# MattJBorowski1991/QuantizedMHA

Measured on AMD Instinct MI355X. Metric: attention-fwd TFLOPS + ms/call, B16 H16 N4096 d64 (fp16 & int8), higher is better.
Workload: dtype int8; 1 GPU; fa_tc_int8_b attention forward (BASELINE config 4); variant=fa_tc_int8_b, B_per_gpu=16, H=16, N=4096, d=64, d_model=1024, global_batch=16, parallelism=batch-shard x1 (no collective in the timed step; all-gather reported separately)

## Files before the change

### include/launchers.h

```cpp
#ifndef QMHA_LAUNCHERS_H
#define QMHA_LAUNCHERS_H

#include <stddef.h>
#include <stdint.h>

#ifdef __cplusplus
extern "C" {
#endif

typedef enum {
    QMHA_FA = 0,
    QMHA_FA_TC_V1A = 1,
    QMHA_FA_TC_INT8_B = 2,
    QMHA_UNFUSED = 3,
    QMHA_FA_MFMA = 4,
    QMHA_FA_TC_INT8_PT = 5
} qmha_variant_t;

enum {
    QMHA_OK = 0,
    QMHA_ERR_INVALID = 1,
    QMHA_ERR_HIP = 2,
    QMHA_ERR_NOMEM = 3,
    QMHA_ERR_NOSYS = 4
// ... 23 lines not shown
                       int variant);

int qmha_quantize_int8(const float *X, int B, int N, int d_model, int h, int8_t *Xi, float *scales, int layout,
                       void *stream);

int qmha_debug_qk_int32(const float *Q, const float *K, int N, int d_model, int h, int head, int32_t *S);

int qmha_debug_fa_int8_dump(const float *Q, const float *K, const float *V, float *O, int B, int N, int d_model,
                            int h, int32_t *S, int8_t *Qi, float *sQ);

int qmha_debug_fa_int8_pt_dump(const float *Q, const float *K, const float *V, float *O, int B, int N, int d_model,
                               int h, int32_t *S, int8_t *Qi, float *sQ);

int64_t qmha_debug_set_pt_wait(int64_t ticks);

int qmha_variant_from_name(const char *name);
const char *qmha_variant_name(int variant);
const char *qmha_status_string(int status);
const char *qmha_version(void);
const char *qmha_last_error(void);

void qmha_profile_enable(int on);
int qmha_set_overlap_chunks(int n);
int qmha_profile_collect(double *main_ms, long long *launches, double *prepass_ms);

void qmha_release_workspaces(void);

#ifdef __cplusplus
}
#endif
#endif
```

### quantizedmha_amd/_lib.py

```python
from __future__ import annotations

import ctypes
import os
import threading

HERE = os.path.dirname(os.path.abspath(__file__))
LIB_DIR = os.path.join(HERE, "lib")
LIB_PATH = os.environ.get("QMHA_LIB_PATH") or os.path.join(LIB_DIR, "libqmha.so")

VARIANTS = {"fa": 0, "fa_tc_v1a": 1, "fa_tc_int8_b": 2, "unfused": 3, "fa_mfma": 4, "fa_tc_int8_pt": 5}
DEFAULT_KERNEL = "fa_tc_int8_b"
QMHA_OK = 0
QMHA_FLAG_CAUSAL = 1

_i, _sz, _vp, _cp = ctypes.c_int, ctypes.c_size_t, ctypes.c_void_p, ctypes.c_char_p
SIGNATURES = {
    "solve": (None, [_vp, _vp, _vp, _vp, _i, _i, _i]),
    "qmha_solve_ex": (_i, [_vp, _vp, _vp, _vp, _i, _i, _i, _i, _i, _vp]),
    "qmha_solve_opts": (_i, [_vp, _vp, _vp, _vp, _i, _i, _i, _i, _i, ctypes.c_uint, _vp, _sz, _vp]),
    "qmha_solve_rect": (_i, [_vp, _vp, _vp, _vp, _i, _i, _i, _i, _i, _i, ctypes.c_uint, _vp, _sz, _vp]),
    "qmha_workspace_size": (_sz, [_i, _i, _i, _i, _i]),
    "qmha_solve_ws": (_i, [_vp, _vp, _vp, _vp, _i, _i, _i, _i, _i, _vp, _sz, _vp]),
    "qmha_solve_variant": (_i, [_vp, _vp, _vp, _vp, _i, _i, _i, _i]),
    "qmha_quantize_int8": (_i, [_vp, _i, _i, _i, _i, _vp, _vp, _i, _vp]),
    "qmha_debug_qk_int32": (_i, [_vp, _vp, _i, _i, _i, _i, _vp]),
    "qmha_debug_fa_int8_dump": (_i, [_vp, _vp, _vp, _vp, _i, _i, _i, _i, _vp, _vp, _vp]),
    "qmha_debug_fa_int8_pt_dump": (_i, [_vp, _vp, _vp, _vp, _i, _i, _i, _i, _vp, _vp, _vp]),
    "qmha_variant_from_name": (_i, [_cp]),
    "qmha_variant_name": (_cp, [_i]),
    "qmha_status_string": (_cp, [_i]),
    "qmha_version": (_cp, []),
    "qmha_last_error": (_cp, []),
    "qmha_profile_enable": (None, [_i]),
    "qmha_set_overlap_chunks": (_i, [_i]),
    "qmha_debug_set_pt_wait": (ctypes.c_longlong, [ctypes.c_longlong]),
    "qmha_profile_collect": (_i, [ctypes.POINTER(ctypes.c_double), ctypes.POINTER(ctypes.c_longlong),
                                  ctypes.POINTER(ctypes.c_double)]),
    "qmha_release_workspaces": (None, []),
}

_lock = threading.Lock()
_lib = None


class QMHAError(RuntimeError):
    pass


def load(path: str = LIB_PATH):
    global _lib
    with _lock:
        if _lib is None:
            if not os.path.exists(path):
                raise QMHAError(f"native library {path} not found: run `python tools/build.py` "
                                "(quantizedmha_amd has no non-HIP fallback)")
            lib = ctypes.CDLL(path)
            for name, (res, args) in SIGNATURES.items():
# ... 18 lines not shown
```

### quantizedmha_amd/csrc/qmha_api.cpp

```cpp
#include <hip/hip_runtime.h>

#include <atomic>
#include <cstdio>
#include <cstdlib>
#include <cstring>
#include <map>
#include <memory>
#include <mutex>
#include <string>
#include <thread>
#include <utility>
#include <vector>

#include "../../include/launchers.h"
#include "qmha_kernels.hpp"

#define QMHA_VERSION_STRING "qmha-mi355x 0.1.0 (gfx950)"

namespace {

thread_local std::string g_last_error;

int fail(int status, std::string why) {
    g_last_error = std::move(why);
// ... 122 lines not shown
int timed(Marks* marks, hipStream_t s, const char* what, Launch&& launch) {
    int st = marks ? mark(*marks, s, true) : QMHA_OK;
    if (st != QMHA_OK) return st;
    QMHA_HIP_TRY(launch(), what);
    return marks ? mark(*marks, s, false) : QMHA_OK;
}

struct WsKey {
    int dev;
    void* stream;
    std::thread::id tid;
    bool operator<(const WsKey& o) const {
        if (dev != o.dev) return dev < o.dev;
        if (stream != o.stream) return stream < o.stream;
        return tid < o.tid;
    }
};
struct WsSlot {
    std::mutex lease;
    void* ptr = nullptr;
    size_t bytes = 0;
    std::vector<std::pair<void*, hipEvent_t>> retired;
    hipStream_t side = nullptr;
    hipEvent_t start = nullptr;
    std::vector<hipEvent_t> ready;
};
std::mutex g_ws_mu;
std::map<WsKey, std::unique_ptr<WsSlot>> g_ws;

void reap_retired(WsSlot& s, bool wait) {
    auto it = s.retired.begin();
    while (it != s.retired.end()) {
        if (wait) (void)hipEventSynchronize(it->second);
        else if (hipEventQuery(it->second) != hipSuccess) {
            ++it;
            continue;
        }
        (void)hipEventDestroy(it->second);
        (void)hipFree(it->first);
        it = s.retired.erase(it);
    }
}

struct WsLease {
    std::unique_lock<std::mutex> lk;
    WsSlot* slot = nullptr;
    void* ptr = nullptr;
// ... 21 lines not shown
            const hipError_t e = hipEventRecord(ev, stream);
            if (e != hipSuccess) {
                (void)hipEventDestroy(ev);
                return hip_fail(e, "hipEventRecord");
            }
            s.retired.emplace_back(s.ptr, ev);
            s.ptr = nullptr;
            s.bytes = 0;
        }
        const size_t alloc = qmha::align_up(need + need / 8, 1 << 20);
        if (hipMalloc(&s.ptr, alloc) != hipSuccess) {
            s.ptr = nullptr;
            return fail(QMHA_ERR_NOMEM, "hipMalloc of workspace failed");
        }
        s.bytes = alloc;
    }
    out->ptr = s.ptr;
    return QMHA_OK;
}

constexpr int kMaxChunks = 16;
std::atomic<int> g_overlap_chunks{-1};

int clamp_chunks(int c) { return c < 1 ? 1 : (c > kMaxChunks ? kMaxChunks : c); }

int overlap_chunks(int B) {
    int c = g_overlap_chunks.load();
    if (c < 0) {
#ifdef QMHA_ABLATION
        const char* e = std::getenv("QMHA_OVERLAP_CHUNKS");
        c = clamp_chunks(e ? std::atoi(e) : 1);
#else
        c = 1;
#endif
        g_overlap_chunks.store(c);
    }
    return c > B ? B : c;
}

int ensure_side(WsSlot& s, int nchunks) {
    if (!s.side) QMHA_HIP_TRY(hipStreamCreateWithFlags(&s.side, hipStreamNonBlocking), "hipStreamCreate");
    if (!s.start) QMHA_HIP_TRY(hipEventCreateWithFlags(&s.start, hipEventDisableTiming), "hipEventCreate");
    while ((int)s.ready.size() < nchunks) {
        hipEvent_t e = nullptr;
        QMHA_HIP_TRY(hipEventCreateWithFlags(&e, hipEventDisableTiming), "hipEventCreate");
        s.ready.push_back(e);
    }
    return QMHA_OK;
}

struct Chunk {
    size_t b0;
    int nb;
};

template <class Pre, class Main>
int run_chunked(int B, hipStream_t stream, WsSlot& slot, Marks* pre_m, Marks* main_m, const char* pre_what, Pre&& pre,
                const char* main_what, Main&& main) {
    const int nc = overlap_chunks(B);
    hipStream_t pre_s = stream;
    if (nc > 1) {
        int st = ensure_side(slot, nc);
        if (st != QMHA_OK) return st;
        QMHA_HIP_TRY(hipEventRecord(slot.start, stream), "hipEventRecord");
        QMHA_HIP_TRY(hipStreamWaitEvent(slot.side, slot.start, 0), "hipStreamWaitEvent");
        pre_s = slot.side;
    }
    Chunk ch[kMaxChunks];
    for (int c = 0; c < nc; ++c) {
        const long long b0 = (long long)B * c / nc, b1 = (long long)B * (c + 1) / nc;
        ch[c] = Chunk{(size_t)b0, (int)(b1 - b0)};
        int st = timed(pre_m, pre_s, pre_what, [&] { return pre(ch[c], pre_s); });
        if (st != QMHA_OK) return st;
        if (nc > 1) QMHA_HIP_TRY(hipEventRecord(slot.ready[c], pre_s), "hipEventRecord");
    }
    for (int c = 0; c < nc; ++c) {
        if (nc > 1) QMHA_HIP_TRY(hipStreamWaitEvent(stream, slot.ready[c], 0), "hipStreamWaitEvent");
        int st = timed(main_m, stream, main_what, [&] { return main(ch[c]); });
        if (st != QMHA_OK) return st;
    }
    return QMHA_OK;
}

qmha::Int8Workspace int8_slice(qmha::Int8Workspace w, size_t b0, int N, int H, int D) {
    const size_t e = b0 * H * N * D, g = b0 * H * (N / 32);
    w.Ki += e, w.Vh += e, w.sK += g, w.sV += g;
    return w;
}
qmha::F16Workspace f16_slice(qmha::F16Workspace w, size_t b0, int N, int H, int D) {
    const size_t e = b0 * H * N * D;
    w.Kh += e, w.Vt += e;
    return w;
}

int run(const float* Q, const float* K, const float* V, float* O, int B, int Nq, int N, int d_model, int h, int variant,
        unsigned flags, void* ws, WsSlot& slot, hipStream_t stream) {
    const int D = d_model / h;
    const bool causal = flags & QMHA_FLAG_CAUSAL;
    const bool rect = Nq != N;
    const bool masked = causal || rect;
    bool prof;
    {
        std::lock_guard<std::mutex> lk(g_prof_mu);
        prof = g_prof_on;
    }
    ProfRec rec;
    Marks *pre_m = prof ? &rec.pre : nullptr, *main_m = prof ? &rec.main : nullptr;
    const size_t slab = (size_t)N * d_model, qslab = (size_t)Nq * d_model;
    int st;
    switch (variant) {
        case QMHA_FA_TC_INT8_B: {
            const qmha::Int8Workspace w8 = qmha::int8_carve(ws, B, N, h, D);
            st = run_chunked(
                B, stream, slot, pre_m, main_m, "quant_int8 launch",
                [&](Chunk c, hipStream_t s) {
                    const qmha::Int8Workspace w = int8_slice(w8, c.b0, N, h, D);
                    return qmha::launch_quant_int8(Q + c.b0 * qslab, K + c.b0 * slab, V + c.b0 * slab, w, w.Vh, 1,
                                                   c.nb, N, h, D, d_model, s, 1);
                },
                rect ? "fa_int8 rect launch" : causal ? "fa_int8 causal launch" : "fa_int8 launch",
                [&](Chunk c) {
                    const qmha::Int8Workspace w = int8_slice(w8, c.b0, N, h, D);
                    const float* q = Q + c.b0 * qslab;
                    float* o = O + c.b0 * qslab;
                    return masked ? qmha::launch_fa_int8_masked_main(w, q, o, c.nb, Nq, N, h, D, d_model, causal, stream)
                                  : qmha::launch_fa_int8_main(w, q, o, c.nb, N, h, D, d_model, stream);
                });
            break;
        }
        case QMHA_FA_TC_V1A: {
            const qmha::F16Workspace w16 = qmha::f16_carve(ws, B, N, h, D);
            st = run_chunked(
                B, stream, slot, pre_m, main_m, "convert_f16 launch",
                [&](Chunk c, hipStream_t s) {
                    return qmha::launch_convert_f16(Q + c.b0 * qslab, K + c.b0 * slab, V + c.b0 * slab,
                                                    f16_slice(w16, c.b0, N, h, D), c.nb, N, h, D, d_model, s);
                },
                rect ? "fa_f16 rect launch" : causal ? "fa_f16 causal launch" : "fa_f16 launch",
                [&](Chunk c) {
                    const qmha::F16Workspace w = f16_slice(w16, c.b0, N, h, D);
                    const float* q = Q + c.b0 * qslab;
                    float* o = O + c.b0 * qslab;
                    return masked ? qmha::launch_fa_f16_masked_main(w, q, o, c.nb, Nq, N, h, D, d_model, causal, stream)
                                  : qmha::launch_fa_f16_main(w, q, o, c.nb, N, h, D, d_model, stream);
                });
            break;
        }
        case QMHA_FA_TC_INT8_PT: {
            const qmha::Int8Workspace w = qmha::int8_pt_carve(ws, B, N, h, D);
            st = timed(pre_m, stream, "quant_int8_pt launch",
                       [&] { return qmha::launch_quant_int8_pt(Q, K, V, w, B, N, h, D, d_model, stream); });
            if (st == QMHA_OK)
                st = timed(main_m, stream, "fa_int8_pt launch",
                           [&] { return qmha::launch_fa_int8_pt_main(w, Q, O, B, N, h, D, d_model, stream); });
            break;
        }
        case QMHA_FA:
        case QMHA_FA_MFMA:
            st = timed(main_m, stream, "fa_f32 launch",
                       [&] { return qmha::launch_fa_f32(Q, K, V, O, B, N, h, D, d_model, variant == QMHA_FA_MFMA, stream); });
            break;
        case QMHA_UNFUSED:
            st = timed(main_m, stream, "unfused launch",
                       [&] { return qmha::launch_unfused(Q, K, V, O, ws, B, N, h, D, d_model, stream); });
            break;
        default: return fail(QMHA_ERR_INVALID, "unknown variant");
    }
// ... 130 lines not shown
            return fail(QMHA_ERR_NOSYS, "layout 2 (per-tensor scales) is built for d = " + d_list(have) + " only");
        WsLease ws;
        st = lease_workspace(qmha::pt_slice_sync_bytes(B, h), (hipStream_t)stream, &ws);
        if (st != QMHA_OK) return st;
        qmha::Int8Workspace w{};
        w.Ki = Xi;
        w.sK = scales;
        w.slice_sync = static_cast<uint32_t*>(ws.ptr);
        QMHA_HIP_TRY(qmha::launch_quant_int8_pt_rows(X, w, B, N, h, D, d_model, (hipStream_t)stream), "quant_int8_pt launch");
        return QMHA_OK;
    }
    qmha::Int8Workspace w{};
    void* vout = nullptr;
    int v_mode = 1, role = 0;
    if (layout == 0) {
        w.Qi = Xi;
        w.sQ = scales;
    } else {
        vout = Xi;
        v_mode = 0;
        w.sV = scales;
        role = 2;
    }
    QMHA_HIP_TRY(qmha::launch_quant_int8(X, X, X, w, vout, v_mode, B, N, h, D, d_model, (hipStream_t)stream, role, 1),
                 "quant_int8 launch");
    return QMHA_OK;
}

int qmha_debug_qk_int32(const float* Q, const float* K, int N, int d_model, int h, int head, int32_t* S) {
    int D = 0;
    int st = check_shape(Q, K, Q, S, 1, N, d_model, h, QMHA_FA_TC_INT8_B, &D);
    if (st != QMHA_OK) return st;
    if (head < 0 || head >= h) return fail(QMHA_ERR_INVALID, "head out of range");
    return debug_run(qmha::int8_workspace_bytes(1, N, h, D, true), [&](void* ws) -> int {
        const qmha::Int8Workspace w = qmha::int8_carve(ws, 1, N, h, D, true);
        QMHA_HIP_TRY(qmha::launch_quant_int8(Q, K, Q, w, w.Vh, 1, 1, N, h, D, d_model, nullptr), "quant_int8 launch");
        QMHA_HIP_TRY(qmha::launch_debug_qk_int32(w, N, D, head, S, nullptr), "debug_qk launch");
        return QMHA_OK;
    });
}

int qmha_debug_fa_int8_dump(const float* Q, const float* K, const float* V, float* O, int B, int N, int d_model,
                            int h, int32_t* S, int8_t* Qi, float* sQ) {
    int D = 0;
    int st = check_shape(Q, K, V, O, B, N, d_model, h, QMHA_FA_TC_INT8_B, &D);
    if (st != QMHA_OK) return st;
    if (!S || !Qi || !sQ || ((D == 32 || D == 64 || D == 128) && N < 64))
// ... 34 lines not shown
const char* qmha_variant_name(int v) {
    const VariantRow* r = find_variant(v);
    return r ? r->name : "unknown";
}

const char* qmha_status_string(int s) {
    switch (s) {
        case QMHA_OK: return "ok";
        case QMHA_ERR_INVALID: return "invalid argument";
        case QMHA_ERR_HIP: return "HIP error";
        case QMHA_ERR_NOMEM: return "out of device memory";
        case QMHA_ERR_NOSYS: return "not supported";
        default: return "unknown status";
    }
}

const char* qmha_version(void) { return QMHA_VERSION_STRING; }

const char* qmha_last_error(void) { return g_last_error.c_str(); }

int64_t qmha_debug_set_pt_wait(int64_t ticks) { return qmha::set_pt_wait_ticks(ticks); }

int qmha_set_overlap_chunks(int n) {
    const int prev = overlap_chunks(1 << 30);
    g_overlap_chunks.store(clamp_chunks(n));
    return prev;
}

void qmha_profile_enable(int on) {
    std::lock_guard<std::mutex> lk(g_prof_mu);
    g_prof_on = on != 0;
}

int qmha_profile_collect(double* main_ms, long long* launches, double* prepass_ms) {
    std::vector<ProfRec> recs;
    {
        std::lock_guard<std::mutex> lk(g_prof_mu);
        recs.swap(g_prof_recs);
    }
    double tm = 0.0, tp = 0.0;
    for (auto& r : recs) {
        for (auto* v : {&r.main, &r.pre}) {
            for (auto& pr : *v) {
                QMHA_HIP_TRY(hipEventSynchronize(pr.second), "hipEventSynchronize");
                float a = 0.0f;
                QMHA_HIP_TRY(hipEventElapsedTime(&a, pr.first, pr.second), "hipEventElapsedTime");
                (v == &r.main ? tm : tp) += a;
            }
        }
    }
// ... 2 lines not shown
        for (auto& r : recs)
            for (auto* v : {&r.main, &r.pre})
                for (auto& pr : *v) {
                    g_event_pool.push_back(pr.first);
                    g_event_pool.push_back(pr.second);
                }
    }
    if (main_ms) *main_ms = tm;
    if (prepass_ms) *prepass_ms = tp;
    if (launches) *launches = (long long)recs.size();
    return QMHA_OK;
}

void qmha_release_workspaces(void) {
    std::lock_guard<std::mutex> lk(g_ws_mu);
    for (auto& kv : g_ws) {
        WsSlot& s = *kv.second;
        std::lock_guard<std::mutex> lease(s.lease);
        (void)hipDeviceSynchronize();
        reap_retired(s, true);
        if (s.ptr) (void)hipFree(s.ptr);
        s.ptr = nullptr;
        s.bytes = 0;
        if (s.side) (void)hipStreamSynchronize(s.side);
        for (hipEvent_t e : s.ready) (void)hipEventDestroy(e);
        s.ready.clear();
        if (s.start) (void)hipEventDestroy(s.start);
        if (s.side) (void)hipStreamDestroy(s.side);
        s.start = nullptr;
        s.side = nullptr;
    }
}

#ifndef QMHA_NO_DEFAULT_SOLVE
void solve(const float* Q, const float* K, const float* V, float* output, int N, int d_model, int h) {
    int st = qmha_solve_variant(Q, K, V, output, N, d_model, h, QMHA_FA_TC_INT8_B);
    if (st != QMHA_OK) std::fprintf(stderr, "qmha solve(fa_tc_int8_b): %s: %s\n", qmha_status_string(st), qmha_last_error());
}
#endif

}
```

### quantizedmha_amd/csrc/qmha_kernels.hpp

```cpp
#pragma once

#include <hip/hip_runtime.h>
#include <math.h>
#include <stddef.h>
#include <stdint.h>

namespace qmha {

inline constexpr size_t align_up(size_t x, size_t a) { return (x + a - 1) / a * a; }

inline constexpr float kLog2e = 1.4426950408889634f;
inline float softmax_scale_log2(int D) { return (1.0f / sqrtf((float)D)) * kLog2e; }

struct Carver {
    char* base;
    size_t used = 0;
    template <class T>
    T* take(size_t bytes) {
        T* p = base ? reinterpret_cast<T*>(base + used) : nullptr;
        used += bytes;
        return p;
    }
};

// ... 10 lines not shown
    size_t bytes;
};
inline Int8Workspace int8_carve(void* ws, int B, int N, int H, int D, bool with_q = false) {
    const size_t e = align_up((size_t)B * H * N * D, 256);
    const size_t s = align_up((size_t)B * H * (N / 32) * sizeof(float), 256);
    Carver c{static_cast<char*>(ws)};
    Int8Workspace w{};
    w.Ki = c.take<int8_t>(e);
    w.Vh = c.take<_Float16>(2 * e);
    w.sK = c.take<float>(s);
    w.sV = c.take<float>(s);
    if (with_q) {
        w.Qi = c.take<int8_t>(e);
        w.sQ = c.take<float>(s);
    }
    w.bytes = c.used;
    return w;
}
inline size_t int8_workspace_bytes(int B, int N, int H, int D, bool with_q = false) {
    return int8_carve(nullptr, B, N, H, D, with_q).bytes;
}
hipError_t launch_quant_int8(const float* Q, const float* K, const float* V, const Int8Workspace& w, void* vout,
                             int v_mode, int B, int N, int H, int D, int d_model, hipStream_t stream,
                             int first_tensor = 0, int num_tensors = -1);
inline size_t pt_slice_sync_bytes(int B, int H) { return align_up((size_t)6 * B * H * sizeof(uint32_t), 256); }
inline Int8Workspace int8_pt_carve(void* ws, int B, int N, int H, int D) {
    const size_t e = align_up((size_t)B * H * N * D, 256);
    const size_t s = align_up((size_t)B * H * sizeof(float), 256);
    Carver c{static_cast<char*>(ws)};
    Int8Workspace w{};
    w.Ki = c.take<int8_t>(e);
    w.Vh = c.take<_Float16>(2 * e);
    w.slice_sync = c.take<uint32_t>(pt_slice_sync_bytes(B, H));
    w.sQ = c.take<float>(s);
    w.sK = c.take<float>(s);
    w.sV = c.take<float>(s);
    w.bytes = c.used;
    return w;
}
inline size_t int8_pt_workspace_bytes(int B, int N, int H, int D) { return int8_pt_carve(nullptr, B, N, H, D).bytes; }
long long set_pt_wait_ticks(long long ticks);
hipError_t launch_quant_int8_pt(const float* Q, const float* K, const float* V, const Int8Workspace& w, int B, int N,
                                int H, int D, int d_model, hipStream_t stream);
hipError_t launch_quant_int8_pt_rows(const float* X, const Int8Workspace& w, int B, int N, int H, int D, int d_model,
                                     hipStream_t stream);
hipError_t launch_fa_int8_pt_main(const Int8Workspace& w, const float* Qf, float* O, int B, int N, int H, int D,
                                  int d_model, hipStream_t stream);
// ... 47 lines not shown
```

### quantizedmha_amd/csrc/qmha_prepass.hip

```cpp
#include <atomic>

#include "qmha_common.hpp"
#include "qmha_kernels.hpp"

namespace qmha {

#ifndef QMHA_PRE_NT
#define QMHA_PRE_NT 1
#endif
#if QMHA_PRE_NT
#define QMHA_PRE_LOAD(p) __builtin_nontemporal_load(p)
#else
#define QMHA_PRE_LOAD(p) (*(p))
#endif
template <int D, int VMODE>
__device__ __forceinline__ void quant_v_group(const float* __restrict__ V, void* __restrict__ Vout,
                                              float* __restrict__ sV, char* vtr, int lane, int b, int k, int g,
                                              int bh, int N, int G, int d_model) {
    constexpr int C4 = D / 4, NI = 32 / (64 / C4);
    const int rq = lane / C4, c4 = lane % C4;
    v4f x[NI];
    float amax = 0.0f;
    const float* base = V + ((size_t)b * N + (size_t)g * QMHA_GROUP) * d_model + (size_t)k * D + 4 * c4;
#pragma unroll
    for (int i = 0; i < NI; ++i) {
        x[i] = QMHA_PRE_LOAD(reinterpret_cast<const v4f*>(base + (size_t)(NI * rq + i) * d_model));
#pragma unroll
        for (int c = 0; c < 4; ++c) amax = fmaxf(amax, fabsf(x[i][c]));
    }
    const float sc = qmha_scale_from_absmax(wave_max64(amax));
    const float inv = 1.0f / sc;
    if constexpr (VMODE == 1)
        vt_group_store<D, true>(vtr, x, inv, lane, static_cast<char*>(Vout) + ((size_t)bh * G + g) * (size_t)(64 * D));
    else
        vt8_group_store<D>(vtr, x, inv, lane, static_cast<char*>(Vout) + ((size_t)bh * G + g) * (size_t)(32 * D));
    if (lane == 0) sV[(size_t)bh * G + g] = sc;
}

template <int D>
__device__ __forceinline__ void quant_row_group(const float* __restrict__ X, int8_t* __restrict__ Xi,
                                                float* __restrict__ sX, int lane, int b, int k, int g, int bh, int N,
                                                int G, int d_model) {
    constexpr int C4 = D / 4, RPI = 64 / C4, NI = 32 / RPI;
    const int ri = lane / C4, ci = lane % C4;
    v4f v[NI];
    float amax = 0.0f;
    const float* base = X + ((size_t)b * N + (size_t)g * QMHA_GROUP) * d_model + (size_t)k * D + 4 * ci;
#pragma unroll
    for (int i = 0; i < NI; ++i) {
        v[i] = QMHA_PRE_LOAD(reinterpret_cast<const v4f*>(base + (size_t)(i * RPI + ri) * d_model));
#pragma unroll
        for (int c = 0; c < 4; ++c) amax = fmaxf(amax, fabsf(v[i][c]));
    }
    const float sc = qmha_scale_from_absmax(wave_max64(amax));
    const float inv = 1.0f / sc;
    int8_t* dst = Xi + ((size_t)bh * N + (size_t)g * QMHA_GROUP) * D + 4 * ci;
#pragma unroll
    for (int i = 0; i < NI; ++i) {
        uint32_t w = 0;
#pragma unroll
        for (int c = 0; c < 4; ++c) w |= ((uint32_t)(uint8_t)qmha_quant_i8(v[i][c], inv)) << (8 * c);
        *reinterpret_cast<uint32_t*>(dst + (size_t)(i * RPI + ri) * D) = w;
    }
    if (lane == 0) sX[(size_t)bh * G + g] = sc;
}

template <int D, int VMODE>
__global__ __launch_bounds__(256) void qmha_quant_int8_kernel(
    const float* __restrict__ Q, const float* __restrict__ K, const float* __restrict__ V,
    int8_t* __restrict__ Qi, int8_t* __restrict__ Ki, void* __restrict__ Vout,
    float* __restrict__ sQ, float* __restrict__ sK, float* __restrict__ sV,
    int N, int H, int d_model, int total_groups, int first_tensor) {
    __shared__ __attribute__((aligned(16))) char vtr[4][D * QMHA_VT_PITCH];
    const int tensor = blockIdx.y + first_tensor;
    const int lane = threadIdx.x & 63;
    const int wave = threadIdx.x >> 6;
    const int item = blockIdx.x * 4 + wave;
    if (item >= total_groups) return;
    const int G = N / QMHA_GROUP;
    const int bh = item / G, g = item % G;
    const int b = bh / H, k = bh % H;
    if (tensor == 2)
        quant_v_group<D, VMODE>(V, Vout, sV, vtr[wave], lane, b, k, g, bh, N, G, d_model);
    else
        quant_row_group<D>(tensor == 0 ? Q : K, tensor == 0 ? Qi : Ki, tensor == 0 ? sQ : sK, lane, b, k, g, bh, N, G,
                           d_model);
}

template <int D>
__global__ __launch_bounds__(256) void qmha_convert_f16_kernel(
    const float* __restrict__ Q, const float* __restrict__ K, const float* __restrict__ V,
    _Float16* __restrict__ Qh, _Float16* __restrict__ Kh, _Float16* __restrict__ Vt,
    int N, int H, int d_model, int total_groups, int first_tensor) {
    constexpr int C4 = D / 4, RPI = 64 / C4, NI = 32 / RPI;
    const int tensor = blockIdx.y + first_tensor;
    const int lane = threadIdx.x & 63, wave = threadIdx.x >> 6;
    const int item = blockIdx.x * 4 + wave;
    const bool active = item < total_groups;
    const int G = N / QMHA_GROUP;
    const int bh = active ? item / G : 0, g = active ? item % G : 0;
    const int b = bh / H, k = bh % H;
    const float* X = tensor == 0 ? Q : (tensor == 1 ? K : V);
    if (tensor == 2) {
        __shared__ __attribute__((aligned(16))) char vtr[4][D * QMHA_VT_PITCH];
        if (active) {
            const int rq = lane / C4, c4 = lane % C4;
            const float* base = V + ((size_t)b * N + (size_t)g * QMHA_GROUP) * d_model + (size_t)k * D + 4 * c4;
            v4f x[NI];
#pragma unroll
            for (int i = 0; i < NI; ++i)
                x[i] = __builtin_nontemporal_load(reinterpret_cast<const v4f*>(base + (size_t)(NI * rq + i) * d_model));
            vt_group_store<D, false>(vtr[wave], x, 1.0f, lane,
// ... 93 lines not shown
    }
    __builtin_amdgcn_s_waitcnt(0xc07f);
    __builtin_amdgcn_wave_barrier();
    char* dst = static_cast<char*>(Vout) + ((size_t)bh * G + g) * (size_t)(VB * D);
    constexpr int LINES = D * VB / 16;
#pragma unroll
    for (int u = lane; u < LINES; u += 64) *reinterpret_cast<v4i*>(dst + 16 * u) = *reinterpret_cast<const v4i*>(T + 16 * u);
}

template <int D, int VMODE, bool QUANT>
static hipError_t prepass_any_d(const float* Q, const float* K, const float* V, void* Qo, void* Ko, void* Vout, float* sQ,
                                float* sK, float* sV, int B, int N, int H, int d_model, int first_tensor, int num_tensors,
                                hipStream_t stream) {
    const int total = B * H * (N / QMHA_GROUP);
    dim3 grid((total + 3) / 4, num_tensors > 0 ? num_tensors : 3 - first_tensor);
    hipLaunchKernelGGL((qmha_prepass_any_kernel<D, VMODE, QUANT>), grid, dim3(256), 0, stream, Q, K, V, Qo, Ko, Vout, sQ, sK,
                       sV, N, H, d_model, total, first_tensor);
    return hipGetLastError();
}

template <int D>
static hipError_t quant_int8_d(const float* Q, const float* K, const float* V, const Int8Workspace& w, void* vout,
                               int v_mode, int B, int N, int H, int d_model, int first_tensor, int num_tensors,
                               hipStream_t stream) {
    const int total = B * H * (N / QMHA_GROUP);
    dim3 grid((total + 3) / 4, num_tensors > 0 ? num_tensors : 3 - first_tensor);
    if (v_mode == 0)
        hipLaunchKernelGGL((qmha_quant_int8_kernel<D, 0>), grid, dim3(256), 0, stream, Q, K, V, w.Qi, w.Ki, vout, w.sQ,
                           w.sK, w.sV, N, H, d_model, total, first_tensor);
    else
        hipLaunchKernelGGL((qmha_quant_int8_kernel<D, 1>), grid, dim3(256), 0, stream, Q, K, V, w.Qi, w.Ki, vout, w.sQ,
                           w.sK, w.sV, N, H, d_model, total, first_tensor);
    return hipGetLastError();
}

__global__ __launch_bounds__(256) void qmha_zero_u32_kernel(uint32_t* __restrict__ p, int n) {
    const int i = blockIdx.x * 256 + threadIdx.x;
    if (i < n) p[i] = 0u;
}

__device__ __forceinline__ void publish_max(uint32_t* mx, float m) {
    const uint32_t old = __hip_atomic_fetch_max(mx, __float_as_uint(m), __ATOMIC_RELAXED, __HIP_MEMORY_SCOPE_AGENT);
    asm volatile("s_waitcnt vmcnt(0)" ::"v"(old) : "memory");
}

constexpr int kPtWaves = 12;
__device__ __forceinline__ float wg_max(const float (&pm)[kPtWaves]) {
    float m = pm[0];
#pragma unroll
    for (int i = 1; i < kPtWaves; ++i) m = fmaxf(m, pm[i]);
// ... 199 lines not shown

hipError_t launch_quant_int8_pt_rows(const float* X, const Int8Workspace& w, int B, int N, int H, int D, int d_model,
                                     hipStream_t stream) {
    switch (D) {
        case 32: return quant_int8_pt_rows_d<32>(X, w, B, N, H, d_model, stream);
        case 64: return quant_int8_pt_rows_d<64>(X, w, B, N, H, d_model, stream);
        case 128: return quant_int8_pt_rows_d<128>(X, w, B, N, H, d_model, stream);
        default: return hipErrorInvalidValue;
    }
}

hipError_t launch_quant_int8_pt(const float* Q, const float* K, const float* V, const Int8Workspace& w, int B, int N,
                                int H, int D, int d_model, hipStream_t stream) {
    switch (D) {
        case 32: return quant_int8_pt_d<32>(Q, K, V, w, B, N, H, d_model, stream);
        case 64: return quant_int8_pt_d<64>(Q, K, V, w, B, N, H, d_model, stream);
        case 128: return quant_int8_pt_d<128>(Q, K, V, w, B, N, H, d_model, stream);
        default: return hipErrorInvalidValue;
    }
}

hipError_t launch_quant_int8(const float* Q, const float* K, const float* V, const Int8Workspace& w, void* vout,
                             int v_mode, int B, int N, int H, int D, int d_model, hipStream_t stream, int first_tensor,
                             int num_tensors) {
    if (first_tensor < 0 || first_tensor > 2 || (num_tensors > 0 && first_tensor + num_tensors > 3))
        return hipErrorInvalidValue;
    switch (D) {
        case 32: return quant_int8_d<32>(Q, K, V, w, vout, v_mode, B, N, H, d_model, first_tensor, num_tensors, stream);
        case 64: return quant_int8_d<64>(Q, K, V, w, vout, v_mode, B, N, H, d_model, first_tensor, num_tensors, stream);
        case 128: return quant_int8_d<128>(Q, K, V, w, vout, v_mode, B, N, H, d_model, first_tensor, num_tensors, stream);
#define QMHA_CASE(d)                                                                                                      \
    case d:                                                                                                               \
        return v_mode == 0 ? prepass_any_d<d, 0, true>(Q, K, V, w.Qi, w.Ki, vout, w.sQ, w.sK, w.sV, B, N, H, d_model,     \
                                                       first_tensor, num_tensors, stream)                                \
                           : prepass_any_d<d, 1, true>(Q, K, V, w.Qi, w.Ki, vout, w.sQ, w.sK, w.sV, B, N, H, d_model,     \
                                                       first_tensor, num_tensors, stream);
        QMHA_CASE(96) QMHA_CASE(160) QMHA_CASE(192) QMHA_CASE(224) QMHA_CASE(256)
#undef QMHA_CASE
        default: return hipErrorInvalidValue;
    }
}


template <int D>
static hipError_t convert_f16_d(const float* Q, const float* K, const float* V, const F16Workspace& w, int B, int N,
                                int H, int d_model, hipStream_t stream) {
    const int total = B * H * (N / QMHA_GROUP);
    hipLaunchKernelGGL((qmha_convert_f16_kernel<D>), dim3((total + 3) / 4, 2), dim3(256), 0, stream, Q, K, V, (_Float16*)nullptr,
                       w.Kh, w.Vt, N, H, d_model, total, 1);
    return hipGetLastError();
}

hipError_t launch_convert_f16(const float* Q, const float* K, const float* V, const F16Workspace& w, int B, int N,
// ... 15 lines not shown
```

Baseline: 785.4 TFLOPS.

## Auto-schedule uneven chunked prepass/main overlap with capped persistent quant kernel

Adds an automatic overlap plan for the int8 FA variant: the batch is split into a small first chunk and larger later chunks. Later quantization prepasses run on a side stream through a new grid-capped persistent loop kernel (about half the CUs, double-buffered loads), so they can share the GPU with attention work. Main attention launches alternate between the caller stream and a second side stream, with a join event at the end. The intent is to hide the quantization prepass behind attention compute, at the cost of more streams and events and possible contention for CUs between concurrent kernels.

```diff
diff --git a/include/launchers.h b/include/launchers.h
--- a/include/launchers.h
+++ b/include/launchers.h
@@ -69,6 +69,8 @@
 
 void qmha_profile_enable(int on);
 int qmha_set_overlap_chunks(int n);
+int qmha_overlap_plan(int variant, int B, int N, int H, int D, int cus, int capturing, int *sizes, int max);
+int qmha_debug_set_prepass_max_wgs(int max_wgs);
 int qmha_profile_collect(double *main_ms, long long *launches, double *prepass_ms);
 
 void qmha_release_workspaces(void);
diff --git a/quantizedmha_amd/_lib.py b/quantizedmha_amd/_lib.py
--- a/quantizedmha_amd/_lib.py
+++ b/quantizedmha_amd/_lib.py
@@ -33,6 +33,8 @@
     "qmha_last_error": (_cp, []),
     "qmha_profile_enable": (None, [_i]),
     "qmha_set_overlap_chunks": (_i, [_i]),
+    "qmha_overlap_plan": (_i, [_i, _i, _i, _i, _i, _i, _i, ctypes.POINTER(_i), _i]),
+    "qmha_debug_set_prepass_max_wgs": (_i, [_i]),
     "qmha_debug_set_pt_wait": (ctypes.c_longlong, [ctypes.c_longlong]),
     "qmha_profile_collect": (_i, [ctypes.POINTER(ctypes.c_double), ctypes.POINTER(ctypes.c_longlong),
                                   ctypes.POINTER(ctypes.c_double)]),
diff --git a/quantizedmha_amd/csrc/qmha_api.cpp b/quantizedmha_amd/csrc/qmha_api.cpp
--- a/quantizedmha_amd/csrc/qmha_api.cpp
+++ b/quantizedmha_amd/csrc/qmha_api.cpp
@@ -168,7 +168,9 @@
     size_t bytes = 0;
     std::vector<std::pair<void*, hipEvent_t>> retired;
     hipStream_t side = nullptr;
+    hipStream_t side2 = nullptr;
     hipEvent_t start = nullptr;
+    hipEvent_t join = nullptr;
     std::vector<hipEvent_t> ready;
 };
 std::mutex g_ws_mu;
@@ -236,9 +238,9 @@
 constexpr int kMaxChunks = 16;
 std::atomic<int> g_overlap_chunks{-1};
 
-int clamp_chunks(int c) { return c < 1 ? 1 : (c > kMaxChunks ? kMaxChunks : c); }
-
-int overlap_chunks(int B) {
+int clamp_chunks(int c) { return c < 0 ? 0 : (c > kMaxChunks ? kMaxChunks : c); }
+
+int overlap_setting() {
     int c = g_overlap_chunks.load();
     if (c < 0) {
 #ifdef QMHA_ABLATION
@@ -249,12 +251,113 @@
 #endif
         g_overlap_chunks.store(c);
     }
-    return c > B ? B : c;
+    return c;
+}
+
+std::atomic<int> g_debug_max_wgs{0};
+int prepass_cap(int planned) {
+    const int forced = g_debug_max_wgs.load(std::memory_order_relaxed);
+    return forced > 0 ? forced : planned;
+}
+
+constexpr int kAutoChunks = 2;
+constexpr int kAutoFirst16 = 1;
+constexpr int kAutoCapHalfCus = 1;
+constexpr int kAutoMinRounds = 8;
+
+struct AutoKnobs {
+    int chunks, first16, cap_half_cus, min_rounds;
+    bool last_on_caller;
+};
+AutoKnobs auto_knobs() {
+    AutoKnobs k{kAutoChunks, kAutoFirst16, kAutoCapHalfCus, kAutoMinRounds, false};
+#ifdef QMHA_ABLATION
+    if (const char* e = std::getenv("QMHA_OVL_CHUNKS")) k.chunks = std::atoi(e);
+    if (const char* e = std::getenv("QMHA_OVL_FIRST16")) k.first16 = std::atoi(e);
+    if (const char* e = std::getenv("QMHA_OVL_CAPH")) k.cap_half_cus = std::atoi(e);
+    if (const char* e = std::getenv("QMHA_OVL_MINROUNDS")) k.min_rounds = std::atoi(e);
+    if (const char* e = std::getenv("QMHA_OVL_LAST_ON_CALLER")) k.last_on_caller = std::atoi(e) != 0;
+#endif
+    return k;
+}
+
+int overlap_plan(int variant, int B, int N, int H, int D, int cus, int capturing, int* sizes, int max) {
+    int plan[kMaxChunks] = {B};
+    int nc = 1;
+    const AutoKnobs k = auto_knobs();
+    const long long wgs = (long long)B * H * ((N + 127) / 128);
+    if (variant == QMHA_FA_TC_INT8_B && D == 64 && B >= 4 && !capturing && cus > 0 &&
+        wgs >= (long long)k.min_rounds * 3 * cus && k.chunks >= 2) {
+        nc = k.chunks > kMaxChunks ? kMaxChunks : k.chunks;
+        if (nc > B) nc = B;
+        int first = (B * k.first16 + 8) / 16;
+        if (first < 1) first = 1;
+        if (first > B - (nc - 1)) first = B - (nc - 1);
+        plan[0] = first;
+        const int rest = B - first;
+        for (int c = 1; c < nc; ++c)
+            plan[c] = (int)((long long)rest * c / (nc - 1) - (long long)rest * (c - 1) / (nc - 1));
+    }
+    if (sizes && max >= 1 && nc > max) {
+        for (int c = max; c < nc; ++c) plan[max - 1] += plan[c];
+        nc = max;
+    }
+    if (sizes)
+        for (int c = 0; c < nc && c < max; ++c) sizes[c] = plan[c];
+    return nc;
+}
+
+int device_cus() {
+    static std::atomic<int> cache[64];
+    int dev = 0;
+    if (hipGetDevice(&dev) != hipSuccess || dev < 0 || dev >= 64) return 0;
+    int c = cache[dev].load(std::memory_order_relaxed);
+    if (c <= 0) {
+        if (hipDeviceGetAttribute(&c, hipDeviceAttributeMultiprocessorCount, dev) != hipSuccess || c <= 0) return 0;
+        cache[dev].store(c, std::memory_order_relaxed);
+    }
+    return c;
+}
+
+struct Schedule {
+    int nc;
+    int sizes[kMaxChunks];
+    int cap;
+    bool last_on_caller = false;
+};
+
+Schedule make_schedule(int variant, int B, int N, int H, int D, bool masked, hipStream_t stream) {
+    Schedule sc{1, {B}, 0};
+    const int setting = overlap_setting();
+    if (setting == 1 || B < 2) return sc;
+    const int cus = device_cus();
+    sc.cap = cus * auto_knobs().cap_half_cus / 2;
+    sc.last_on_caller = auto_knobs().last_on_caller;
+    if (setting >= 2) {
+        sc.nc = setting > B ? B : setting;
+        for (int c = 0; c < sc.nc; ++c) sc.sizes[c] = (int)((long long)B * (c + 1) / sc.nc - (long long)B * c / sc.nc);
+        return sc;
+    }
+    if (masked) return sc;
+    int sizes[kMaxChunks];
+    const int nc = overlap_plan(variant, B, N, H, D, cus, 0, sizes, kMaxChunks);
+    if (nc < 2) return sc;
+    hipStreamCaptureStatus cap = hipStreamCaptureStatusNone;
+    if (hipStreamIsCapturing(stream, &cap) != hipSuccess) {
+        (void)hipGetLastError();
+        return sc;
+    }
+    if (cap != hipStreamCaptureStatusNone) return sc;
+    sc.nc = nc;
+    for (int c = 0; c < nc; ++c) sc.sizes[c] = sizes[c];
+    return sc;
 }
 
 int ensure_side(WsSlot& s, int nchunks) {
     if (!s.side) QMHA_HIP_TRY(hipStreamCreateWithFlags(&s.side, hipStreamNonBlocking), "hipStreamCreate");
+    if (!s.side2) QMHA_HIP_TRY(hipStreamCreateWithFlags(&s.side2, hipStreamNonBlocking), "hipStreamCreate");
     if (!s.start) QMHA_HIP_TRY(hipEventCreateWithFlags(&s.start, hipEventDisableTiming), "hipEventCreate");
+    if (!s.join) QMHA_HIP_TRY(hipEventCreateWithFlags(&s.join, hipEventDisableTiming), "hipEventCreate");
     while ((int)s.ready.size() < nchunks) {
         hipEvent_t e = nullptr;
         QMHA_HIP_TRY(hipEventCreateWithFlags(&e, hipEventDisableTiming), "hipEventCreate");
@@ -269,31 +372,44 @@
 };
 
 template <class Pre, class Main>
-int run_chunked(int B, hipStream_t stream, WsSlot& slot, Marks* pre_m, Marks* main_m, const char* pre_what, Pre&& pre,
-                const char* main_what, Main&& main) {
-    const int nc = overlap_chunks(B);
-    hipStream_t pre_s = stream;
-    if (nc > 1) {
-        int st = ensure_side(slot, nc);
+int run_chunked(const Schedule& sc, hipStream_t stream, WsSlot& slot, Marks* pre_m, Marks* main_m, const char* pre_what,
+                Pre&& pre, const char* main_what, Main&& main) {
+    const int nc = sc.nc;
+    Chunk ch[kMaxChunks];
+    size_t b0 = 0;
+    for (int c = 0; c < nc; ++c) {
+        ch[c] = Chunk{b0, sc.sizes[c]};
+        b0 += (size_t)sc.sizes[c];
+    }
+    const int cap0 = prepass_cap(0);
+    if (nc == 1) {
+        int st = timed(pre_m, stream, pre_what, [&] { return pre(ch[0], stream, cap0); });
         if (st != QMHA_OK) return st;
-        QMHA_HIP_TRY(hipEventRecord(slot.start, stream), "hipEventRecord");
-        QMHA_HIP_TRY(hipStreamWaitEvent(slot.side, slot.start, 0), "hipStreamWaitEvent");
-        pre_s = slot.side;
-    }
-    Chunk ch[kMaxChunks];
+        return timed(main_m, stream, main_what, [&] { return main(ch[0], stream); });
+    }
+    int st = ensure_side(slot, nc);
+    if (st != QMHA_OK) return st;
+    QMHA_HIP_TRY(hipEventRecord(slot.start, stream), "hipEventRecord");
+    QMHA_HIP_TRY(hipStreamWaitEvent(slot.side, slot.start, 0), "hipStreamWaitEvent");
+    st = timed(pre_m, stream, pre_what, [&] { return pre(ch[0], stream, cap0); });
+    if (st != QMHA_OK) return st;
+    const int cap = prepass_cap(sc.cap);
+    for (int c = 1; c < nc; ++c) {
+        st = timed(pre_m, slot.side, pre_what, [&] { return pre(ch[c], slot.side, cap); });
+        if (st != QMHA_OK) return st;
+        QMHA_HIP_TRY(hipEventRecord(slot.ready[c], slot.side), "hipEventRecord");
+    }
+    if (main_m && (st = mark(*main_m, stream, true)) != QMHA_OK) return st;
+    const int flip = sc.last_on_caller ? (nc - 1) & 1 : 0;
+    if (flip) QMHA_HIP_TRY(hipEventRecord(slot.ready[0], stream), "hipEventRecord");
     for (int c = 0; c < nc; ++c) {
-        const long long b0 = (long long)B * c / nc, b1 = (long long)B * (c + 1) / nc;
-        ch[c] = Chunk{(size_t)b0, (int)(b1 - b0)};
-        int st = timed(pre_m, pre_s, pre_what, [&] { return pre(ch[c], pre_s); });
-        if (st != QMHA_OK) return st;
-        if (nc > 1) QMHA_HIP_TRY(hipEventRecord(slot.ready[c], pre_s), "hipEventRecord");
-    }
-    for (int c = 0; c < nc; ++c) {
-        if (nc > 1) QMHA_HIP_TRY(hipStreamWaitEvent(stream, slot.ready[c], 0), "hipStreamWaitEvent");
-        int st = timed(main_m, stream, main_what, [&] { return main(ch[c]); });
-        if (st != QMHA_OK) return st;
-    }
-    return QMHA_OK;
+        hipStream_t s = ((c ^ flip) & 1) ? slot.side2 : stream;
+        if (c > 0 || flip) QMHA_HIP_TRY(hipStreamWaitEvent(s, slot.ready[c], 0), "hipStreamWaitEvent");
+        QMHA_HIP_TRY(main(ch[c], s), main_what);
+    }
+    QMHA_HIP_TRY(hipEventRecord(slot.join, slot.side2), "hipEventRecord");
+    QMHA_HIP_TRY(hipStreamWaitEvent(stream, slot.join, 0), "hipStreamWaitEvent");
+    return main_m ? mark(*main_m, stream, false) : QMHA_OK;
 }
 
 qmha::Int8Workspace int8_slice(qmha::Int8Workspace w, size_t b0, int N, int H, int D) {
@@ -322,41 +438,43 @@
     Marks *pre_m = prof ? &rec.pre : nullptr, *main_m = prof ? &rec.main : nullptr;
     const size_t slab = (size_t)N * d_model, qslab = (size_t)Nq * d_model;
     int st;
+    const bool chunked = variant == QMHA_FA_TC_INT8_B || variant == QMHA_FA_TC_V1A;
+    const Schedule sched = chunked ? make_schedule(variant, B, N, h, D, masked, stream) : Schedule{1, {B}, 0};
     switch (variant) {
         case QMHA_FA_TC_INT8_B: {
             const qmha::Int8Workspace w8 = qmha::int8_carve(ws, B, N, h, D);
             st = run_chunked(
-                B, stream, slot, pre_m, main_m, "quant_int8 launch",
-                [&](Chunk c, hipStream_t s) {
+                sched, stream, slot, pre_m, main_m, "quant_int8 launch",
+                [&](Chunk c, hipStream_t s, int max_wgs) {
                     const qmha::Int8Workspace w = int8_slice(w8, c.b0, N, h, D);
                     return qmha::launch_quant_int8(Q + c.b0 * qslab, K + c.b0 * slab, V + c.b0 * slab, w, w.Vh, 1,
-                                                   c.nb, N, h, D, d_model, s, 1);
+                                                   c.nb, N, h, D, d_model, s, 1, -1, max_wgs);
                 },
                 rect ? "fa_int8 rect launch" : causal ? "fa_int8 causal launch" : "fa_int8 launch",
-                [&](Chunk c) {
+                [&](Chunk c, hipStream_t s) {
                     const qmha::Int8Workspace w = int8_slice(w8, c.b0, N, h, D);
                     const float* q = Q + c.b0 * qslab;
                     float* o = O + c.b0 * qslab;
-                    return masked ? qmha::launch_fa_int8_masked_main(w, q, o, c.nb, Nq, N, h, D, d_model, causal, stream)
-                                  : qmha::launch_fa_int8_main(w, q, o, c.nb, N, h, D, d_model, stream);
+                    return masked ? qmha::launch_fa_int8_masked_main(w, q, o, c.nb, Nq, N, h, D, d_model, causal, s)
+                                  : qmha::launch_fa_int8_main(w, q, o, c.nb, N, h, D, d_model, s);
                 });
             break;
         }
         case QMHA_FA_TC_V1A: {
             const qmha::F16Workspace w16 = qmha::f16_carve(ws, B, N, h, D);
             st = run_chunked(
-                B, stream, slot, pre_m, main_m, "convert_f16 launch",
-                [&](Chunk c, hipStream_t s) {
+                sched, stream, slot, pre_m, main_m, "convert_f16 launch",
+                [&](Chunk c, hipStream_t s, int ) {
                     return qmha::launch_convert_f16(Q + c.b0 * qslab, K + c.b0 * slab, V + c.b0 * slab,
                                                     f16_slice(w16, c.b0, N, h, D), c.nb, N, h, D, d_model, s);
                 },
                 rect ? "fa_f16 rect launch" : causal ? "fa_f16 causal launch" : "fa_f16 launch",
-                [&](Chunk c) {
+                [&](Chunk c, hipStream_t s) {
                     const qmha::F16Workspace w = f16_slice(w16, c.b0, N, h, D);
                     const float* q = Q + c.b0 * qslab;
                     float* o = O + c.b0 * qslab;
-                    return masked ? qmha::launch_fa_f16_masked_main(w, q, o, c.nb, Nq, N, h, D, d_model, causal, stream)
-                                  : qmha::launch_fa_f16_main(w, q, o, c.nb, N, h, D, d_model, stream);
+                    return masked ? qmha::launch_fa_f16_masked_main(w, q, o, c.nb, Nq, N, h, D, d_model, causal, s)
+                                  : qmha::launch_fa_f16_main(w, q, o, c.nb, N, h, D, d_model, s);
                 });
             break;
         }
@@ -533,7 +651,8 @@
         w.sV = scales;
         role = 2;
     }
-    QMHA_HIP_TRY(qmha::launch_quant_int8(X, X, X, w, vout, v_mode, B, N, h, D, d_model, (hipStream_t)stream, role, 1),
+    QMHA_HIP_TRY(qmha::launch_quant_int8(X, X, X, w, vout, v_mode, B, N, h, D, d_model, (hipStream_t)stream, role, 1,
+                                         prepass_cap(0)),
                  "quant_int8 launch");
     return QMHA_OK;
 }
@@ -614,10 +733,17 @@
 int64_t qmha_debug_set_pt_wait(int64_t ticks) { return qmha::set_pt_wait_ticks(ticks); }
 
 int qmha_set_overlap_chunks(int n) {
-    const int prev = overlap_chunks(1 << 30);
+    const int prev = overlap_setting();
     g_overlap_chunks.store(clamp_chunks(n));
     return prev;
 }
+
+int qmha_overlap_plan(int variant, int B, int N, int H, int D, int cus, int capturing, int* sizes, int max) {
+    if (B < 1 || N < 1 || H < 1 || D < 1) return 0;
+    return overlap_plan(variant, B, N, H, D, cus, capturing, sizes, max);
+}
+
+int qmha_debug_set_prepass_max_wgs(int max_wgs) { return g_debug_max_wgs.exchange(max_wgs > 0 ? max_wgs : 0); }
 
 void qmha_profile_enable(int on) {
     std::lock_guard<std::mutex> lk(g_prof_mu);
@@ -666,13 +792,18 @@
         if (s.ptr) (void)hipFree(s.ptr);
         s.ptr = nullptr;
         s.bytes = 0;
-        if (s.side) (void)hipStreamSynchronize(s.side);
+        for (hipStream_t side : {s.side, s.side2})
+            if (side) (void)hipStreamSynchronize(side);
         for (hipEvent_t e : s.ready) (void)hipEventDestroy(e);
         s.ready.clear();
-        if (s.start) (void)hipEventDestroy(s.start);
-        if (s.side) (void)hipStreamDestroy(s.side);
-        s.start = nullptr;
-        s.side = nullptr;
+        for (hipEvent_t* e : {&s.start, &s.join}) {
+            if (*e) (void)hipEventDestroy(*e);
+            *e = nullptr;
+        }
+        for (hipStream_t* side : {&s.side, &s.side2}) {
+            if (*side) (void)hipStreamDestroy(*side);
+            *side = nullptr;
+        }
     }
 }
 
diff --git a/quantizedmha_amd/csrc/qmha_kernels.hpp b/quantizedmha_amd/csrc/qmha_kernels.hpp
--- a/quantizedmha_amd/csrc/qmha_kernels.hpp
+++ b/quantizedmha_amd/csrc/qmha_kernels.hpp
@@ -56,7 +56,7 @@
 }
 hipError_t launch_quant_int8(const float* Q, const float* K, const float* V, const Int8Workspace& w, void* vout,
                              int v_mode, int B, int N, int H, int D, int d_model, hipStream_t stream,
-                             int first_tensor = 0, int num_tensors = -1);
+                             int first_tensor = 0, int num_tensors = -1, int max_wgs = 0);
 inline size_t pt_slice_sync_bytes(int B, int H) { return align_up((size_t)6 * B * H * sizeof(uint32_t), 256); }
 inline Int8Workspace int8_pt_carve(void* ws, int B, int N, int H, int D) {
     const size_t e = align_up((size_t)B * H * N * D, 256);
diff --git a/quantizedmha_amd/csrc/qmha_prepass.hip b/quantizedmha_amd/csrc/qmha_prepass.hip
--- a/quantizedmha_amd/csrc/qmha_prepass.hip
+++ b/quantizedmha_amd/csrc/qmha_prepass.hip
@@ -13,18 +13,23 @@
 #else
 #define QMHA_PRE_LOAD(p) (*(p))
 #endif
-template <int D, int VMODE>
-__device__ __forceinline__ void quant_v_group(const float* __restrict__ V, void* __restrict__ Vout,
-                                              float* __restrict__ sV, char* vtr, int lane, int b, int k, int g,
-                                              int bh, int N, int G, int d_model) {
+template <int D>
+__device__ __forceinline__ void quant_v_load(v4f (&x)[D / 8], const float* __restrict__ V, int lane, int b, int k, int g,
+                                             int N, int d_model) {
     constexpr int C4 = D / 4, NI = 32 / (64 / C4);
     const int rq = lane / C4, c4 = lane % C4;
-    v4f x[NI];
+    const float* base = V + ((size_t)b * N + (size_t)g * QMHA_GROUP) * d_model + (size_t)k * D + 4 * c4;
+#pragma unroll
+    for (int i = 0; i < NI; ++i)
+        x[i] = QMHA_PRE_LOAD(reinterpret_cast<const v4f*>(base + (size_t)(NI * rq + i) * d_model));
+}
+template <int D, int VMODE>
+__device__ __forceinline__ void quant_v_finish(const v4f (&x)[D / 8], void* __restrict__ Vout, float* __restrict__ sV,
+                                               char* vtr, int lane, int g, int bh, int G) {
+    constexpr int NI = D / 8;
     float amax = 0.0f;
-    const float* base = V + ((size_t)b * N + (size_t)g * QMHA_GROUP) * d_model + (size_t)k * D + 4 * c4;
 #pragma unroll
     for (int i = 0; i < NI; ++i) {
-        x[i] = QMHA_PRE_LOAD(reinterpret_cast<const v4f*>(base + (size_t)(NI * rq + i) * d_model));
 #pragma unroll
         for (int c = 0; c < 4; ++c) amax = fmaxf(amax, fabsf(x[i][c]));
     }
@@ -36,33 +41,55 @@
         vt8_group_store<D>(vtr, x, inv, lane, static_cast<char*>(Vout) + ((size_t)bh * G + g) * (size_t)(32 * D));
     if (lane == 0) sV[(size_t)bh * G + g] = sc;
 }
-
+template <int D, int VMODE>
+__device__ __forceinline__ void quant_v_group(const float* __restrict__ V, void* __restrict__ Vout,
+                                              float* __restrict__ sV, char* vtr, int lane, int b, int k, int g,
+                                              int bh, int N, int G, int d_model) {
+    v4f x[D / 8];
+    quant_v_load<D>(x, V, lane, b, k, g, N, d_model);
+    quant_v_finish<D, VMODE>(x, Vout, sV, vtr, lane, g, bh, G);
+}
+
+template <int D>
+__device__ __forceinline__ void quant_row_load(v4f (&v)[D / 8], const float* __restrict__ X, int lane, int b, int k, int g,
+                                               int N, int d_model) {
+    constexpr int C4 = D / 4, RPI = 64 / C4, NI = 32 / RPI;
+    const int ri = lane / C4, ci = lane % C4;
+    const float* base = X + ((size_t)b * N + (size_t)g * QMHA_GROUP) * d_model + (size_t)k * D + 4 * ci;
+#pragma unroll
+    for (int i = 0; i < NI; ++i)
+        v[i] = QMHA_PRE_LOAD(reinterpret_cast<const v4f*>(base + (size_t)(i * RPI + ri) * d_model));
+}
+template <int D>
+__device__ __forceinline__ void quant_row_finish(const v4f (&v)[D / 8], int8_t* __restrict__ Xi, float* __restrict__ sX,
+                                                 int lane, int g, int bh, int N, int G) {
+    constexpr int C4 = D / 4, RPI = 64 / C4, NI = 32 / RPI;
+    const int ri = lane / C4, ci = lane % C4;
+    float amax = 0.0f;
+#pragma unroll
+    for (int i = 0; i < NI; ++i) {
+#pragma unroll
+        for (int c = 0; c < 4; ++c) amax = fmaxf(amax, fabsf(v[i][c]));
+    }
+    const float sc = qmha_scale_from_absmax(wave_max64(amax));
+    const float inv = 1.0f / sc;
+    int8_t* dst = Xi + ((size_t)bh * N + (size_t)g * QMHA_GROUP) * D + 4 * ci;
+#pragma unroll
+    for (int i = 0; i < NI; ++i) {
+        uint32_t w = 0;
+#pragma unroll
+        for (int c = 0; c < 4; ++c) w |= ((uint32_t)(uint8_t)qmha_quant_i8(v[i][c], inv)) << (8 * c);
+        *reinterpret_cast<uint32_t*>(dst + (size_t)(i * RPI + ri) * D) = w;
+    }
+    if (lane == 0) sX[(size_t)bh * G + g] = sc;
+}
 template <int D>
 __device__ __forceinline__ void quant_row_group(const float* __restrict__ X, int8_t* __restrict__ Xi,
                                                 float* __restrict__ sX, int lane, int b, int k, int g, int bh, int N,
                                                 int G, int d_model) {
-    constexpr int C4 = D / 4, RPI = 64 / C4, NI = 32 / RPI;
-    const int ri = lane / C4, ci = lane % C4;
-    v4f v[NI];
-    float amax = 0.0f;
-    const float* base = X + ((size_t)b * N + (size_t)g * QMHA_GROUP) * d_model + (size_t)k * D + 4 * ci;
-#pragma unroll
-    for (int i = 0; i < NI; ++i) {
-        v[i] = QMHA_PRE_LOAD(reinterpret_cast<const v4f*>(base + (size_t)(i * RPI + ri) * d_model));
-#pragma unroll
-        for (int c = 0; c < 4; ++c) amax = fmaxf(amax, fabsf(v[i][c]));
-    }
-    const float sc = qmha_scale_from_absmax(wave_max64(amax));
-    const float inv = 1.0f / sc;
-    int8_t* dst = Xi + ((size_t)bh * N + (size_t)g * QMHA_GROUP) * D + 4 * ci;
-#pragma unroll
-    for (int i = 0; i < NI; ++i) {
-        uint32_t w = 0;
-#pragma unroll
-        for (int c = 0; c < 4; ++c) w |= ((uint32_t)(uint8_t)qmha_quant_i8(v[i][c], inv)) << (8 * c);
-        *reinterpret_cast<uint32_t*>(dst + (size_t)(i * RPI + ri) * D) = w;
-    }
-    if (lane == 0) sX[(size_t)bh * G + g] = sc;
+    v4f v[D / 8];
+    quant_row_load<D>(v, X, lane, b, k, g, N, d_model);
+    quant_row_finish<D>(v, Xi, sX, lane, g, bh, N, G);
 }
 
 template <int D, int VMODE>
@@ -88,6 +115,56 @@
 }
 
 template <int D>
+__global__ __launch_bounds__(256) void qmha_quant_int8_loop_kernel(
+    const float* __restrict__ Q, const float* __restrict__ K, const float* __restrict__ V,
+    int8_t* __restrict__ Qi, int8_t* __restrict__ Ki, void* __restrict__ Vout,
+    float* __restrict__ sQ, float* __restrict__ sK, float* __restrict__ sV,
+    int N, int H, int d_model, int total_groups, int first_tensor, int v_mode) {
+    __shared__ __attribute__((aligned(16))) char vtr[4][D * QMHA_VT_PITCH];
+    constexpr int NI = D / 8;
+    const int tensor = blockIdx.y + first_tensor;
+    const int lane = threadIdx.x & 63;
+    const int wave = threadIdx.x >> 6;
+    const int stride = 4 * gridDim.x;
+    int item = blockIdx.x * 4 + wave;
+    if (item >= total_groups) return;
+    const int G = N / QMHA_GROUP;
+    const float* X = tensor == 0 ? Q : (tensor == 1 ? K : V);
+    auto load = [&](v4f(&x)[NI], int it) {
+        const int bh = it / G, g = it % G;
+        if (tensor == 2) quant_v_load<D>(x, X, lane, bh / H, bh % H, g, N, d_model);
+        else quant_row_load<D>(x, X, lane, bh / H, bh % H, g, N, d_model);
+    };
+    auto finish = [&](const v4f(&x)[NI], int it) {
+        const int bh = it / G, g = it % G;
+        if (tensor == 2) {
+            if (v_mode == 1) quant_v_finish<D, 1>(x, Vout, sV, vtr[wave], lane, g, bh, G);
+            else quant_v_finish<D, 0>(x, Vout, sV, vtr[wave], lane, g, bh, G);
+            __builtin_amdgcn_s_waitcnt(0xc07f);
+            __builtin_amdgcn_wave_barrier();
+        } else {
+            quant_row_finish<D>(x, tensor == 0 ? Qi : Ki, tensor == 0 ? sQ : sK, lane, g, bh, N, G);
+        }
+    };
+    v4f xa[NI], xb[NI];
+    load(xa, item);
+    for (;;) {
+        int next = item + stride;
+        bool more = next < total_groups;
+        if (more) load(xb, next);
+        finish(xa, item);
+        if (!more) break;
+        item = next;
+        next = item + stride;
+        more = next < total_groups;
+        if (more) load(xa, next);
+        finish(xb, item);
+        if (!more) break;
+        item = next;
+    }
+}
+
+template <int D>
 __global__ __launch_bounds__(256) void qmha_convert_f16_kernel(
     const float* __restrict__ Q, const float* __restrict__ K, const float* __restrict__ V,
     _Float16* __restrict__ Qh, _Float16* __restrict__ Kh, _Float16* __restrict__ Vt,
@@ -227,10 +304,14 @@
 template <int D>
 static hipError_t quant_int8_d(const float* Q, const float* K, const float* V, const Int8Workspace& w, void* vout,
                                int v_mode, int B, int N, int H, int d_model, int first_tensor, int num_tensors,
-                               hipStream_t stream) {
+                               int max_wgs, hipStream_t stream) {
     const int total = B * H * (N / QMHA_GROUP);
     dim3 grid((total + 3) / 4, num_tensors > 0 ? num_tensors : 3 - first_tensor);
-    if (v_mode == 0)
+    if (max_wgs > 0) {
+        if ((int)grid.x > max_wgs) grid.x = max_wgs;
+        hipLaunchKernelGGL((qmha_quant_int8_loop_kernel<D>), grid, dim3(256), 0, stream, Q, K, V, w.Qi, w.Ki, vout, w.sQ,
+                           w.sK, w.sV, N, H, d_model, total, first_tensor, v_mode);
+    } else if (v_mode == 0)
         hipLaunchKernelGGL((qmha_quant_int8_kernel<D, 0>), grid, dim3(256), 0, stream, Q, K, V, w.Qi, w.Ki, vout, w.sQ,
                            w.sK, w.sV, N, H, d_model, total, first_tensor);
     else
@@ -476,13 +557,13 @@
 
 hipError_t launch_quant_int8(const float* Q, const float* K, const float* V, const Int8Workspace& w, void* vout,
                              int v_mode, int B, int N, int H, int D, int d_model, hipStream_t stream, int first_tensor,
-                             int num_tensors) {
+                             int num_tensors, int max_wgs) {
     if (first_tensor < 0 || first_tensor > 2 || (num_tensors > 0 && first_tensor + num_tensors > 3))
         return hipErrorInvalidValue;
     switch (D) {
-        case 32: return quant_int8_d<32>(Q, K, V, w, vout, v_mode, B, N, H, d_model, first_tensor, num_tensors, stream);
-        case 64: return quant_int8_d<64>(Q, K, V, w, vout, v_mode, B, N, H, d_model, first_tensor, num_tensors, stream);
-        case 128: return quant_int8_d<128>(Q, K, V, w, vout, v_mode, B, N, H, d_model, first_tensor, num_tensors, stream);
+        case 32: return quant_int8_d<32>(Q, K, V, w, vout, v_mode, B, N, H, d_model, first_tensor, num_tensors, max_wgs, stream);
+        case 64: return quant_int8_d<64>(Q, K, V, w, vout, v_mode, B, N, H, d_model, first_tensor, num_tensors, max_wgs, stream);
+        case 128: return quant_int8_d<128>(Q, K, V, w, vout, v_mode, B, N, H, d_model, first_tensor, num_tensors, max_wgs, stream);
 #define QMHA_CASE(d)                                                                                                      \
     case d:                                                                                                               \
         return v_mode == 0 ? prepass_any_d<d, 0, true>(Q, K, V, w.Qi, w.Ki, vout, w.sQ, w.sK, w.sV, B, N, H, d_model,     \
```

After: 784.9 TFLOPS (median of 2 runs). No clear change (-0.1%).
